# ZwwWayne/mmMOT

Hardware: NVIDIA H100
Metric: frame-pairs/sec at N=128 dets (higher is better)
Workload: dtype f32 (tensor-core engine: FP16 hi/lo split operands, fp32 accumulate)

## Files before the change

### mmmot_b200/csrc/gemm_tma.cuh

```cuda
#pragma once
#include <cuda.h>
#include <cuda_fp16.h>

#include "tc_common.cuh"

namespace tma {

using namespace tc;

constexpr int T_THREADS = 384;
constexpr int T_EPI_WARPS = 8, T_LOAD_WARP = 8;
constexpr int T_CONS_REGS = 232, T_LOAD_REGS = 40;
static_assert(256 * T_CONS_REGS + 128 * T_LOAD_REGS <= launch_regs(T_THREADS) * T_THREADS, "register split exceeds the CTA's pool");
constexpr int T_EPI_SCRATCH = 32 * 80;
constexpr int T_STAGES = 4;
constexpr int T_STAGE_BYTES = A_SUB + 2 * B_HALF;
constexpr size_t T_SMEM_BYTES = (size_t)T_STAGES * T_STAGE_BYTES + 1024 + 256 + T_EPI_WARPS * T_EPI_SCRATCH;
static_assert(T_SMEM_BYTES <= 227 * 1024, "gemm_tma_kernel exceeds the 227 KB of shared memory per block");
static_assert(T_STAGES * T_STAGE_BYTES >= 128 * BN * 4, "the accumulator image must fit in the ring it overlays");

enum { OUT_PLANAR = 3 };

struct TmaP {
  TcP t;
  int conv;
  int bx, by, bi;
  int tiles_x, tiles_y;
  int n_img, H, W, C;
  long plane_elems;
  int ksegs, kc_per_seg;
  float* acc_scratch;
  int halo, pool;
  unsigned long long* pool_sum;
  unsigned long long* segsum;
  int* status;
  int wcompact;
  const float* gen_src;
  const int4* chunk_tab;
};

static __global__ void seg_chunk_tab_kernel(const int4* __restrict__ tiles, int num_tiles, const int* __restrict__ seg,
                                            int4* __restrict__ tab) {
  const int idx = blockIdx.x * blockDim.x + threadIdx.x;
  if (idx >= num_tiles * 2) return;
  const int4 tt = tiles[idx >> 1];
  const int half = idx & 1, c0 = tt.y, len = tt.z;
  int v[4];
#pragma unroll
  for (int c = 0; c < 4; c++) {
    const int col0 = half * 128 + c * 32;
    v[c] = 0;
    if (col0 < len) {
      const int first = seg[c0 + col0], last = seg[c0 + min(col0 + 31, len - 1)];
      v[c] = (first << 1) | ((col0 + 32 <= len && first == last) ? 1 : 0);
    }
  }
  tab[idx] = make_int4(v[0], v[1], v[2], v[3]);
}

__device__ __forceinline__ void tma_load_2d(uint32_t dst, const CUtensorMap* map, int c0, int c1, uint32_t mbar) {
  asm volatile(
      "cp.async.bulk.tensor.2d.shared::cluster.global.tile.mbarrier::complete_tx::bytes [%0], [%1, {%2, %3}], [%4];"
      ::"r"(dst), "l"(reinterpret_cast<uint64_t>(map)), "r"(c0), "r"(c1), "r"(mbar)
      : "memory");
}
__device__ __forceinline__ void tma_load_4d(uint32_t dst, const CUtensorMap* map, int c0, int c1, int c2, int c3,
                                            uint32_t mbar) {
  asm volatile(
      "cp.async.bulk.tensor.4d.shared::cluster.global.tile.mbarrier::complete_tx::bytes [%0], [%1, {%2, %3, %4, %5}], "
      "[%6];"
      ::"r"(dst), "l"(reinterpret_cast<uint64_t>(map)), "r"(c0), "r"(c1), "r"(c2), "r"(c3), "r"(mbar)
      : "memory");
}
__device__ __forceinline__ uint64_t smem_desc_sw64(uint32_t saddr) {
  return (uint64_t)((saddr & 0x3FFFFu) >> 4) | ((uint64_t)1 << 16) | ((uint64_t)(512 >> 4) << 32) | (2ull << 62);
}
__device__ __forceinline__ void st_global_256(void* dst, const uint4& a, const uint4& b) {
  asm volatile("st.global.v4.b32 [%0], {%1, %2, %3, %4};\n\tst.global.v4.b32 [%0+16], {%5, %6, %7, %8};" ::"l"(dst),
               "r"(a.x), "r"(a.y), "r"(a.z), "r"(a.w), "r"(b.x), "r"(b.y), "r"(b.z), "r"(b.w)
               : "memory");
}
__device__ __forceinline__ void st_global_256(void* dst, const uint32_t* r) {
  st_global_256(dst, make_uint4(r[0], r[1], r[2], r[3]), make_uint4(r[4], r[5], r[6], r[7]));
}
__device__ __forceinline__ void split_f16(float x, __half& hi, __half& lo) {
  unsigned short a, b;
  asm("{\n\t.reg .f32 f;\n\t"
      "cvt.rn.satfinite.f16.f32 %0, %2;\n\t"
      "cvt.f32.f16 f, %0;\n\t"
      "sub.f32 f, %2, f;\n\t"
      "cvt.rn.satfinite.f16.f32 %1, f;\n\t}"
      : "=h"(a), "=h"(b)
      : "f"(x));
  hi = __ushort_as_half(a);
  lo = __ushort_as_half(b);
}

template <int BX>
__device__ __forceinline__ void pool_chunk(const float (&x)[32], float (&o)[8]) {
#pragma unroll
  for (int a = 0; a < 16 / BX; a++)
#pragma unroll
    for (int b = 0; b < BX / 2; b++) {
      const int i = 2 * a * BX + 2 * b;
      o[a * (BX / 2) + b] = fmaxf(fmaxf(x[i], x[i + 1]), fmaxf(x[i + BX], x[i + BX + 1]));
    }
}

static __global__ void __launch_bounds__(T_THREADS, 1)
gemm_tma_kernel(const TmaP P, const __grid_constant__ CUtensorMap map_hi, const __grid_constant__ CUtensorMap map_lo) {
  const GemmP& p = P.t.g;
  extern __shared__ uint8_t smem_raw[];
  const uint32_t raw = smem_u32(smem_raw);
  const uint32_t base = (raw + 1023u) & ~1023u;
  uint8_t* sm = smem_raw + (base - raw);
  const uint32_t bar0 = base + T_STAGES * T_STAGE_BYTES;
  auto full_bar = [&](int s) { return bar0 + 8u * s; };
  auto empty_bar = [&](int s) { return bar0 + 8u * (T_STAGES + s); };
  const uint32_t free_bar = bar0 + 8u * (2 * T_STAGES);
  float* img = reinterpret_cast<float*>(sm);
  uint8_t* epi_scratch = sm + T_STAGES * T_STAGE_BYTES + 256;

  const int tid = threadIdx.x, warp = tid >> 5, lane = tid & 31;
  const int mgroups = P.t.m_tiles;
  const long total_tiles = (long)p.num_tiles * mgroups;
  const int KC = P.t.k_chunks;
  const int cchunks = P.conv ? P.C / BK : KC;

  if (tid == 0) {
    for (int s = 0; s < T_STAGES; s++) {
      mbar_init(full_bar(s), 1);
      mbar_init(empty_bar(s), T_EPI_WARPS);
    }
    mbar_init(free_bar, T_EPI_WARPS);
    asm volatile("fence.mbarrier_init.release.cluster;" ::: "memory");
  }
  __syncthreads();

  auto tile_cols = [&](int nt, int& g, int& c0, int& len) {
    if (p.tile_tab) { int4 tt = p.tile_tab[nt]; g = tt.x; c0 = tt.y; len = tt.z; }
    else { g = nt / p.tiles_per_group; c0 = (nt - g * p.tiles_per_group) * BN; len = min(BN, p.S - c0); }
  };
  auto conv_origin = [&](int nt, int& i0, int& y0, int& x0) {
    const int tx = nt % P.tiles_x;
    const int r = nt / P.tiles_x;
    const int ty = r % P.tiles_y;
    i0 = (r / P.tiles_y) * P.bi; y0 = ty * P.by; x0 = tx * P.bx;
  };

  if (warp < T_EPI_WARPS) {
    asm volatile("setmaxnreg.inc.sync.aligned.u32 %0;" ::"n"(T_CONS_REGS));
    const int q = warp & 3, half = warp >> 2;
    const int lbx = 31 - __clz(max(P.bx, 1)), lby = 31 - __clz(max(P.by, 1));
    uint32_t wcount = 0;
    uint32_t it = 0;
    float acc[2][64];
    float amax = 0.f;
    __half* yh = reinterpret_cast<__half*>(p.Y);
    __half* scr = reinterpret_cast<__half*>(epi_scratch + warp * T_EPI_SCRATCH);
    auto store_rows = [&](const float (&x)[32], bool ok, long o) {
      __half h[32], l[32];
#pragma unroll
      for (int j = 0; j < 32; j++) { split_f16(x[j], h[j], l[j]); amax = fmaxf(amax, fabsf(x[j])); }
#pragma unroll
      for (int pl = 0; pl < 2; pl++) {
#pragma unroll
        for (int j = 0; j < 32; j++) scr[j * 40 + lane] = pl ? l[j] : h[j];
        __syncwarp();
        if (ok) {
          const uint4* src = reinterpret_cast<const uint4*>(scr + lane * 40);
          __half* dst = yh + o + (pl ? P.plane_elems : 0);
          const uint4 a = src[0], b = src[1], c = src[2], d = src[3];
          st_global_256(dst, a, b);
          st_global_256(dst + 16, c, d);
        }
        __syncwarp();
      }
    };
    auto store_planar_block = [&](const float (&x)[32], int col0, int cb, int i0, int y0, int x0) {
      const int col = col0 + lane;
      const int xx = col & (P.bx - 1), r = col >> lbx;
      const int yy = r & (P.by - 1), ii = r >> lby;
      const int img = i0 + ii, y = y0 + yy, xg = x0 + xx;
      store_rows(x, img < P.n_img && y < P.H && xg < P.W, (((long)img * P.H + y) * P.W + xg) * p.y_ms + cb);
    };
    const int Hp = P.H >> 1, Wp = P.W >> 1;
    float hprev[16];
    float psum = 0.f;
    int psum_img = -1;
    auto pool_flush = [&](int co_) {
      if (P.pool_sum && psum_img >= 0 && psum_img < P.n_img)
        atomicAdd(P.pool_sum + (long)psum_img * p.M + co_, __float2ull_rn(psum * 4294967296.f));
      psum = 0.f; psum_img = -1;
    };
    auto pool_emit = [&](const float (&o)[16], int np, int r0, int rstep_q, int wq, int cb, int co_, int i0, int y0, int x0) {
      float xs[32];
#pragma unroll
      for (int j = 0; j < 32; j++) xs[j] = j < 16 ? o[j] : 0.f;
      const int q = lane < np ? lane : 0;
      const int r = r0 + 2 * (q / wq), xx = 2 * (q - (q / wq) * wq);
      const int yy = r & (P.by - 1), ii = r >> lby;
      const int img = i0 + ii, y = y0 + yy, xg = x0 + xx;
      const bool ok = lane < np && img < P.n_img && y < P.H && xg < P.W;
      store_rows(xs, ok, (((long)img * Hp + (y >> 1)) * Wp + (xg >> 1)) * p.y_ms + cb);
      if (P.pool_sum) {
        (void)rstep_q;
#pragma unroll
        for (int j = 0; j < 16; j++) {
          if (j < np) {
            const int rj = r0 + 2 * (j / wq), xj = 2 * (j - (j / wq) * wq);
            const int imj = i0 + (rj >> lby);
            const bool okj = imj < P.n_img && y0 + (rj & (P.by - 1)) < P.H && x0 + xj < P.W;
            if (imj != psum_img) { pool_flush(co_); psum_img = imj; }
            if (okj) psum += o[j];
          }
        }
      }
    };
    auto emit_conv = [&](const float (&x)[32], int cc, int col0, int co_, int i0, int y0, int x0) {
      if (!P.pool) { store_planar_block(x, col0, co_ - lane, i0, y0, x0); return; }
      float o[16];
      const int r0 = col0 >> lbx;
      if (P.bx == 32) {
        if (!(cc & 1)) {
#pragma unroll
          for (int b = 0; b < 16; b++) hprev[b] = fmaxf(x[2 * b], x[2 * b + 1]);
          return;
        }
#pragma unroll
        for (int b = 0; b < 16; b++) o[b] = fmaxf(hprev[b], fmaxf(x[2 * b], x[2 * b + 1]));
        pool_emit(o, 16, r0 - 1, 0, 16, co_ - lane, co_, i0, y0, x0);
        return;
      }
      float o8[8];
      if (P.bx == 16) pool_chunk<16>(x, o8);
      else if (P.bx == 8) pool_chunk<8>(x, o8);
      else if (P.bx == 4) pool_chunk<4>(x, o8);
      else pool_chunk<2>(x, o8);
#pragma unroll
      for (int j = 0; j < 16; j++) o[j] = j < 8 ? o8[j] : 0.f;
      pool_emit(o, 8, r0, 0, P.bx >> 1, co_ - lane, co_, i0, y0, x0);
    };

    for (long t = blockIdx.x; t < total_tiles; t += gridDim.x) {
      const int mg = (int)(t % mgroups);
      const int nt = (int)(t / mgroups);
      int g = 0, c0 = 0, len = BN, i0 = 0, y0 = 0, x0 = 0;
      if (P.conv) conv_origin(nt, i0, y0, x0); else tile_cols(nt, g, c0, len);
      for (int seg = 0; seg < P.ksegs; seg++, wcount++) {
#pragma unroll
      for (int mb = 0; mb < 2; mb++)
#pragma unroll
        for (int i = 0; i < 64; i++) acc[mb][i] = 0.f;
      const int kc_lo = seg * P.kc_per_seg, kc_hi = min(KC, kc_lo + P.kc_per_seg);
      for (int kc = kc_lo; kc < kc_hi; kc++, it++) {
        const int s = it % T_STAGES;
        mbar_wait(full_bar(s), (it / T_STAGES) & 1);
        const uint32_t sa = base + s * T_STAGE_BYTES, sb = sa + A_SUB + half * (128 / 8) * 512;
        if (!(P.t.dbg & 8)) {
          wgmma_fence();
#pragma unroll
          for (int ks = 0; ks < 2; ks++) {
            const uint64_t b_hi = smem_desc_sw64(sb + ks * 32), b_lo = smem_desc_sw64(sb + B_HALF + ks * 32);
#pragma unroll
            for (int mb = 0; mb < 2; mb++) {
              const uint32_t a = sa + mb * 8 * SBO + ks * 2 * A_LBO;
              const uint64_t a_hi = smem_desc(a, A_LBO, SBO), a_lo = smem_desc(a + A_HALF, A_LBO, SBO);
              wgmma_n128(acc[mb], a_hi, b_hi, ((kc - kc_lo) | ks) ? 1u : 0u);
              wgmma_n128(acc[mb], a_hi, b_lo, 1u);
              wgmma_n128(acc[mb], a_lo, b_hi, 1u);
            }
          }
          wgmma_commit();
        }
        wgmma_wait<1>();
        if (kc > kc_lo) { __syncwarp(); if (lane == 0) mbar_arrive(empty_bar((it - 1) % T_STAGES)); }
      }
      wgmma_wait<0>();
      fence_acc(acc[0]);
      fence_acc(acc[1]);
      __syncwarp();
      if (lane == 0) mbar_arrive(empty_bar((it - 1) % T_STAGES));
      bar_sync(7, T_EPI_WARPS * 32);
      acc_dump(acc[0], img, BN, 0, half * 128);
      acc_dump(acc[1], img, BN, 64, half * 128);
      bar_sync(7, T_EPI_WARPS * 32);
      if (P.ksegs > 1) {
        {
          const int co = mg * 128 + q * 32 + lane;
          const bool rowok = co < p.M;
          const float bv = (rowok && p.bias) ? __ldg(p.bias + co) : 0.f;
#pragma unroll 1
          for (int cc = 0; cc < 4; cc++) {
            const int col0 = half * 128 + cc * 32;
            uint32_t v[32];
            acc_ld32(img, BN, q * 32 + lane, col0, v);
            if (!rowok) continue;
            float* sp = P.acc_scratch + ((long)nt * BN + col0) * p.M + co;
            if (seg < P.ksegs - 1) {
              if (seg == 0) {
#pragma unroll
                for (int j = 0; j < 32; j++) __stcg(sp + (long)j * p.M, __uint_as_float(v[j]) * P.t.out_scale);
              } else {
                float sv[32];
#pragma unroll
                for (int j = 0; j < 32; j++) sv[j] = __ldcg(sp + (long)j * p.M);
#pragma unroll
                for (int j = 0; j < 32; j++) __stcg(sp + (long)j * p.M, fmaf(__uint_as_float(v[j]), P.t.out_scale, sv[j]));
              }
            } else {
              float sv[32];
#pragma unroll
              for (int j = 0; j < 32; j++) sv[j] = __ldcg(sp + (long)j * p.M);
#pragma unroll
              for (int j = 0; j < 32; j++) {
                float a = fmaf(__uint_as_float(v[j]), P.t.out_scale, sv[j]) + bv;
                sv[j] = p.relu ? fmaxf(a, 0.f) : a;
              }
              emit_conv(sv, cc, col0, co, i0, y0, x0);
            }
          }
          if (P.pool && seg == P.ksegs - 1 && rowok) pool_flush(co);
        }
      } else
      {
        const int co = mg * 128 + q * 32 + lane;
        const bool rowok = co < p.M;
        const float bv = (rowok && p.bias) ? __ldg(p.bias + co) : 0.f;
        double f1 = 0.0, f2 = 0.0;
        const bool pass2 = P.segsum && !p.part && !p.Y && !p.relu;
        const bool use_seg = p.seg && (p.addend || P.segsum);
        int4 ct = make_int4(0, 0, 0, 0);
        if (use_seg) ct = __ldg(P.chunk_tab + (long)nt * 2 + half);
        const int cdesc[4] = {ct.x, ct.y, ct.z, ct.w};
        float adv[4] = {0.f, 0.f, 0.f, 0.f};
        unsigned one_det = 0;
#pragma unroll
        for (int c = 0; c < 4; c++) {
          if (cdesc[c] & 1) {
            one_det |= 1u << c;
            if (p.addend && rowok) adv[c] = __ldg(p.addend + (long)(cdesc[c] >> 1) * p.ld_add + co);
          }
        }
        float na = 0.f, nb = 0.f;
        if (P.segsum && rowok) { na = __ldg(p.sc + (long)g * p.M + co); nb = __ldg(p.sh + (long)g * p.M + co); }
#pragma unroll 1
        for (int cc = 0; cc < 4; cc++) {
          const int col0 = half * 128 + cc * 32;
          if (col0 >= len) break;
          const int da = (cc == 0 ? ct.x : cc == 1 ? ct.y : cc == 2 ? ct.z : ct.w) >> 1;
          const float adc = cc == 0 ? adv[0] : cc == 1 ? adv[1] : cc == 2 ? adv[2] : adv[3];
          const bool single = (one_det >> cc) & 1u;
          uint32_t v[32];
          acc_ld32(img, BN, q * 32 + lane, col0, v);
          if (P.t.dbg & 1) continue;
          float s1 = 0.f, s2 = 0.f, pv = 0.f;
          bool fast = col0 + 32 <= len;
          if (pass2 && fast) {
            if (single) {
              if (rowok) {
                const float bva = bv + adc;
                const float a2 = P.t.out_scale * na, b2 = fmaf(bva, na, nb);
                float r0 = 0.f, r1 = 0.f;
#pragma unroll
                for (int j = 0; j < 32; j += 2) {
                  r0 += fmaxf(fmaf(__uint_as_float(v[j]), a2, b2), 0.f);
                  r1 += fmaxf(fmaf(__uint_as_float(v[j + 1]), a2, b2), 0.f);
                }
                atomicAdd(P.segsum + (long)da * p.M + co, __float2ull_rn((r0 + r1) * 4294967296.f));
              }
              continue;
            }
          }
          float bva = bv;
          if (fast && p.addend) {
            if (single) bva += adc;
            else fast = false;
          }
          if (fast) {
            if (p.relu) epi_fast<true>(v, P.t.out_scale, bva, pv, s1, s2);
            else epi_fast<false>(v, P.t.out_scale, bva, pv, s1, s2);
          } else {
            float t = 0.f;
#pragma unroll
            for (int j = 0; j < 32; j++) {
              float x = fmaf(__uint_as_float(v[j]), P.t.out_scale, bv);
              const int col = col0 + j;
              if (p.addend && rowok && col < len)
                x += __ldg(p.addend + (long)__ldg(p.seg + c0 + col) * p.ld_add + co);
              if (p.relu) x = fmaxf(x, 0.f);
              v[j] = __float_as_uint(x);
              if (col < len) t += x;
            }
            pv = t / (float)min(32, len - col0);
#pragma unroll
            for (int j = 0; j < 32; j++)
              if (col0 + j < len) { const float d = __uint_as_float(v[j]) - pv; s1 += d; s2 = fmaf(d, d, s2); }
          }
          stat_fold(f1, f2, min(32, len - col0), pv, s1, s2);
          if (P.segsum && rowok) {
            const int nvalid = min(32, len - col0);
            int dcur = da;
            float run = 0.f;
            if (single) {
#pragma unroll
              for (int j = 0; j < 32; j++) run += fmaxf(fmaf(__uint_as_float(v[j]), na, nb), 0.f);
            } else {
#pragma unroll
              for (int j = 0; j < 32; j++) {
                if (j < nvalid) {
                  const int d = __ldg(p.seg + c0 + col0 + j);
                  if (d != dcur) {
                    atomicAdd(P.segsum + (long)dcur * p.M + co, __float2ull_rn(run * 4294967296.f));
                    run = 0.f; dcur = d;
                  }
                  run += fmaxf(fmaf(__uint_as_float(v[j]), na, nb), 0.f);
                }
              }
            }
            atomicAdd(P.segsum + (long)dcur * p.M + co, __float2ull_rn(run * 4294967296.f));
          }
          if (!p.Y || !rowok) continue;
          if (P.conv) {
            float xv[32];
#pragma unroll
            for (int j = 0; j < 32; j++) xv[j] = __uint_as_float(v[j]);
            emit_conv(xv, cc, col0, co, i0, y0, x0);
          } else {
            const int nvalid = min(32, len - col0);
            const long row0 = (long)g * p.y_gs + c0 + col0;
            if (P.t.out_mode == OUT_PLANAR && !(p.y_ms & 31)) {
              float xv[32];
#pragma unroll
              for (int j = 0; j < 32; j++) xv[j] = __uint_as_float(v[j]);
              store_rows(xv, lane < nvalid, (row0 + lane) * p.y_ms + (co - lane));
            } else if (P.t.out_mode == OUT_PLANAR) {
              __half* dst = yh + row0 * p.y_ms + co;
#pragma unroll
              for (int j = 0; j < 32; j++)
                if (j < nvalid) {
                  __half h, l;
                  split_f16(__uint_as_float(v[j]), h, l);
                  amax = fmaxf(amax, fabsf(__uint_as_float(v[j])));
                  dst[(long)j * p.y_ms] = h;
                  dst[(long)j * p.y_ms + P.plane_elems] = l;
                }
            } else {
              float* dst = p.Y + row0 * p.y_ms + co;
              if (nvalid == 32) {
#pragma unroll
                for (int j = 0; j < 32; j++) { *dst = __uint_as_float(v[j]); dst += p.y_ms; }
              } else {
#pragma unroll
                for (int j = 0; j < 32; j++)
                  if (j < nvalid) dst[(long)j * p.y_ms] = __uint_as_float(v[j]);
              }
            }
          }
        }
        if (p.part && rowok) p.part[((long)nt * 2 + half) * p.M + co] = make_double2(f1, f2);
        if (P.conv && P.pool && rowok) pool_flush(co);
      }
      fence_async_smem();
      __syncwarp();
      if (lane == 0) mbar_arrive(free_bar);
      }
    }
    mm_range_flag(P.status, amax);
  } else {
    asm volatile("setmaxnreg.dec.sync.aligned.u32 %0;" ::"n"(T_LOAD_REGS));
    if (warp == T_LOAD_WARP && lane == 0) {
      uint32_t it = 0, wcount = 0;
      for (long t = blockIdx.x; t < total_tiles; t += gridDim.x) {
        const int mg = (int)(t % mgroups);
        const int nt = (int)(t / mgroups);
        const int mt0 = mg;
        int g = 0, c0 = 0, len = BN, i0 = 0, y0 = 0, x0 = 0;
        if (P.conv) conv_origin(nt, i0, y0, x0); else tile_cols(nt, g, c0, len);
        const int row0 = (int)((long)g * p.x_gs + c0);
        for (int kc = 0; kc < KC; kc++, it++) {
          if (kc % P.kc_per_seg == 0) {
            if (wcount > 0) mbar_wait(free_bar, (wcount - 1) & 1);
            wcount++;
          }
          const int s = it % T_STAGES;
          mbar_wait(empty_bar(s), ((it / T_STAGES) & 1) ^ 1);
          const uint32_t abytes = (uint32_t)A_SUB;
          const bool skipA = P.t.dbg & 2, skipB = P.t.dbg & 4;
          mbar_expect_tx(full_bar(s), (skipA ? 0u : abytes) + (skipB ? 0u : 2u * B_HALF));
          const uint32_t sa = base + s * T_STAGE_BYTES, sb = sa + A_SUB;
          const uint8_t* src = reinterpret_cast<const uint8_t*>(P.t.Wp) + ((size_t)kc * P.t.m_tiles + mt0) * A_SUB;
          if (!skipA) bulk_g2s(sa, src, abytes, full_bar(s));
          if (skipB) continue;
          if (P.conv) {
            const int tap = kc / cchunks, cc = kc - tap * cchunks;
            const int dx = tap % 3 - 1, dy = tap / 3 - 1;
            tma_load_4d(sb, &map_hi, cc * BK, x0 + dx, y0 + dy, i0, full_bar(s));
            tma_load_4d(sb + B_HALF, &map_lo, cc * BK, x0 + dx, y0 + dy, i0, full_bar(s));
          } else {
            tma_load_2d(sb, &map_hi, kc * BK, row0, full_bar(s));
            tma_load_2d(sb + B_HALF, &map_lo, kc * BK, row0, full_bar(s));
          }
        }
      }
    }
    __syncwarp();
  }

}

typedef CUresult (*EncodeTiledFn)(CUtensorMap*, CUtensorMapDataType, cuuint32_t, void*, const cuuint64_t*,
                                  const cuuint64_t*, const cuuint32_t*, const cuuint32_t*, CUtensorMapInterleave,
                                  CUtensorMapSwizzle, CUtensorMapL2promotion, CUtensorMapFloatOOBfill);
static inline EncodeTiledFn encode_fn() {
  static EncodeTiledFn fn = nullptr;
  if (!fn) {
    void* p = nullptr;
    cudaDriverEntryPointQueryResult qr;
    if (cudaGetDriverEntryPoint("cuTensorMapEncodeTiled", &p, cudaEnableDefault, &qr) == cudaSuccess &&
        qr == cudaDriverEntryPointSuccess)
      fn = (EncodeTiledFn)p;
  }
  return fn;
}
static inline int make_map_2d(CUtensorMap* m, const void* basep, long rows, int C, long ld) {
  EncodeTiledFn fn = encode_fn();
  if (!fn) return MMMOT_E_ARG;
  cuuint64_t dims[2] = {(cuuint64_t)C, (cuuint64_t)rows};
  cuuint64_t strides[1] = {(cuuint64_t)ld * 2};
  cuuint32_t box[2] = {32, 256}, es[2] = {1, 1};
  CUresult r = fn(m, CU_TENSOR_MAP_DATA_TYPE_FLOAT16, 2, const_cast<void*>(basep), dims, strides, box, es,
                  CU_TENSOR_MAP_INTERLEAVE_NONE, CU_TENSOR_MAP_SWIZZLE_64B, CU_TENSOR_MAP_L2_PROMOTION_L2_128B,
                  CU_TENSOR_MAP_FLOAT_OOB_FILL_NONE);
  return r == CUDA_SUCCESS ? 0 : 900 + (int)r;
}
static inline int make_map_2d_f32(CUtensorMap* m, const void* basep, long rows, int C, int box_rows,
                                  CUtensorMapSwizzle swizzle) {
  EncodeTiledFn fn = encode_fn();
  if (!fn) return MMMOT_E_ARG;
  cuuint64_t dims[2] = {(cuuint64_t)C, (cuuint64_t)rows};
  cuuint64_t strides[1] = {(cuuint64_t)C * 4};
  cuuint32_t box[2] = {32, (cuuint32_t)box_rows}, es[2] = {1, 1};
  CUresult r = fn(m, CU_TENSOR_MAP_DATA_TYPE_FLOAT32, 2, const_cast<void*>(basep), dims, strides, box, es,
                  CU_TENSOR_MAP_INTERLEAVE_NONE, swizzle, CU_TENSOR_MAP_L2_PROMOTION_L2_128B,
                  CU_TENSOR_MAP_FLOAT_OOB_FILL_NONE);
  return r == CUDA_SUCCESS ? 0 : 900 + (int)r;
}
static inline int make_map_4d(CUtensorMap* m, const void* basep, int n_img, int H, int W, int C, int bx, int by,
                              int bi) {
  EncodeTiledFn fn = encode_fn();
  if (!fn) return MMMOT_E_ARG;
  cuuint64_t dims[4] = {(cuuint64_t)C, (cuuint64_t)W, (cuuint64_t)H, (cuuint64_t)n_img};
  cuuint64_t strides[3] = {(cuuint64_t)C * 2, (cuuint64_t)W * C * 2, (cuuint64_t)H * W * C * 2};
  cuuint32_t box[4] = {32, (cuuint32_t)bx, (cuuint32_t)by, (cuuint32_t)bi}, es[4] = {1, 1, 1, 1};
  CUresult r = fn(m, CU_TENSOR_MAP_DATA_TYPE_FLOAT16, 4, const_cast<void*>(basep), dims, strides, box, es,
                  CU_TENSOR_MAP_INTERLEAVE_NONE, CU_TENSOR_MAP_SWIZZLE_64B, CU_TENSOR_MAP_L2_PROMOTION_L2_128B,
                  CU_TENSOR_MAP_FLOAT_OOB_FILL_NONE);
  return r == CUDA_SUCCESS ? 0 : 900 + (int)r;
}

}

#include "gemm_tma_px.cuh"

static int gemm_tma_px_launch(tma::TmaP& P, const CUtensorMap& mh, const CUtensorMap& ml, int sms, cudaStream_t st) {
  static std::atomic<unsigned long long> attr{0};
  MM_TRY(mm_ensure_smem(tma::gemm_tma_px_kernel<false>, tma::PX_SMEM_BYTES, attr));
  const long total = P.t.g.num_tiles;
  const int grid = (int)(total < sms ? total : sms);
  tma::gemm_tma_px_kernel<false><<<grid, tma::PX_THREADS, tma::PX_SMEM_BYTES, st>>>(P, mh, ml);
  MM_LAUNCH_CHECK();
  return 0;
}

static int gemm_tma_px_launch_gen27(const float* crops, int n_img, int H, int W, const uint4* Wpx, float out_scale,
                                    const float* bias, __half* Yhi, long y_plane, int* status, cudaStream_t st) {
  if (!crops || !Wpx || !Yhi) return MMMOT_E_ARG;
  const long n_pix = (long)n_img * H * W;
  if (n_pix >= (1L << 31) || ((long)H * W) % tc::BN || (tc::BN + 2 * W + 2) * 12 > 2 * tma::PX_W_SLOT) return MMMOT_E_SHAPE;
  int sms = 0;
  MM_TRY(mm_sm_count(&sms));
  static std::atomic<unsigned long long> attr{0};
  MM_TRY(mm_ensure_smem(tma::gemm_tma_px_kernel<true>, tma::PX_SMEM_BYTES, attr));
  tma::TmaP P;
  memset(&P, 0, sizeof(P));
  GemmP g = gemm_defaults();
  g.bias = bias; g.M = 64; g.K = 32; g.relu = 1;
  g.S = (int)n_pix; g.tiles_per_group = mm_cdiv(n_pix, tc::BN); g.num_tiles = g.tiles_per_group;
  g.Y = reinterpret_cast<float*>(Yhi); g.y_ms = 64;
  P.t.g = g;
  P.t.Wp = Wpx; P.wcompact = 1;
  P.t.m_tiles = 1; P.t.k_chunks = 1;
  P.t.out_scale = out_scale;
  P.t.out_mode = tma::OUT_PLANAR;
  P.t.dbg = mm_debug_flags();
  P.plane_elems = y_plane;
  P.ksegs = 1; P.kc_per_seg = 1;
  P.status = status;
  P.gen_src = crops; P.n_img = n_img; P.H = H; P.W = W;
  alignas(64) CUtensorMap dummy;
  memset(&dummy, 0, sizeof(dummy));
  const long total = g.num_tiles;
  const int grid = (int)(total < sms ? total : sms);
  tma::gemm_tma_px_kernel<true><<<grid, tma::PX_GEN_THREADS, tma::PX_SMEM_BYTES, st>>>(P, dummy, dummy);
  MM_LAUNCH_CHECK();
  return 0;
}

static int gemm_tma_launch_mat(const GemmP& g, const uint4* Wp, float out_scale, const __half* Xhi, long x_plane,
                               long rows, int ldx, int out_mode, long y_plane, cudaStream_t st,
                               unsigned long long* segsum = nullptr, int* status = nullptr, const int4* chunk_tab = nullptr,
                               const uint4* Wpx = nullptr) {
  if (!Wp || g.num_tiles <= 0 || g.K % tc::BK) return MMMOT_E_ARG;
  int sms = 0;
  MM_TRY(mm_sm_count(&sms));
  static std::atomic<unsigned long long> attr{0};
  MM_TRY(mm_ensure_smem(tma::gemm_tma_kernel, tma::T_SMEM_BYTES, attr));
  tma::TmaP P;
  memset(&P, 0, sizeof(P));
  P.t.g = g;
  P.t.Wp = Wp;
  P.t.m_tiles = (g.M + 127) / 128;
  P.t.k_chunks = g.K / tc::BK;
  P.t.out_scale = out_scale;
  P.t.out_mode = out_mode;
  P.t.dbg = mm_debug_flags();
  P.plane_elems = y_plane;
  P.ksegs = 1; P.kc_per_seg = P.t.k_chunks;
  P.segsum = segsum;
  P.status = status;
  P.chunk_tab = chunk_tab;
  if (g.seg && (g.addend || segsum) && !chunk_tab) return MMMOT_E_ARG;
  alignas(64) CUtensorMap mh, ml;
  MM_TRY(tma::make_map_2d(&mh, Xhi, rows, g.K, ldx));
  MM_TRY(tma::make_map_2d(&ml, Xhi + x_plane, rows, g.K, ldx));
  if (out_mode == tma::OUT_PLANAR && g.M == 64 && g.y_ms == 64 && !g.part && !segsum && !g.addend && !g.tile_tab &&
      !(P.t.dbg & 64)) {
    if (Wpx) { P.t.Wp = Wpx; P.wcompact = 1; }
    return gemm_tma_px_launch(P, mh, ml, sms, st);
  }
  const long total = (long)g.num_tiles * P.t.m_tiles;
  const int grid = (int)(total < sms ? total : sms);
  tma::gemm_tma_kernel<<<grid, tma::T_THREADS, tma::T_SMEM_BYTES, st>>>(P, mh, ml);
  MM_LAUNCH_CHECK();
  return 0;
}

static inline double conv_box_waste(int n_img, int H, int W, int bx, int by, int bi) {
  return (double)mm_cdiv(W, bx) * bx / W * mm_cdiv(H, by) * by / H * mm_cdiv(n_img, bi) * bi / n_img;
}

struct ConvPlan {
  int px;
  int halo;
  int pool;
  int bx, by, bi;
  int ksegs, kc_per_seg;
  int tiles_x, tiles_y, num_tiles;
};
static inline ConvPlan conv_plan(int M, bool part, int n_img, int H, int W, int C, bool want_pool, bool use_kseg, int dbg,
                                 int seg_chunks) {
  ConvPlan c;
  memset(&c, 0, sizeof(c));
  c.bx = 1; c.by = 1; c.bi = 256;
  double best = 1e30;
  for (int cx = 256; cx >= 1; cx >>= 1)
    for (int cy = 256 / cx; cy >= 1; cy >>= 1) {
      const int ci = 256 / (cx * cy);
      const double waste = conv_box_waste(n_img, H, W, cx, cy, ci);
      if (waste < best - 1e-9) { best = waste; c.bx = cx; c.by = cy; c.bi = ci; }
    }
  const int kchunks = 9 * C / tc::BK;
  c.px = M == 64 && !part && !(dbg & 64) && !(use_kseg && seg_chunks > 0 && kchunks > seg_chunks);
  if (c.px && conv_box_waste(1, H, W, 16, 16, 1) <= best + 1e-9) { c.bx = 16; c.by = 16; c.bi = 1; }
  if (c.px) {
    c.halo = (c.bi == 1 && c.bx >= 8 && c.bx * (c.by + 2) * 64 <= tma::PX_X_PLANE && !(dbg & 256)) ? 1 : 0;
    c.pool = want_pool && c.bx >= 2 && c.bx <= 16 && c.by >= 2 && !(H & 1) && !(W & 1) && !(dbg & 512);
  } else {
    c.pool = want_pool && c.bx >= 2 && c.bx <= 32 && c.by >= 2 && !(H & 1) && !(W & 1) && !(dbg & 512);
  }
  c.ksegs = 1; c.kc_per_seg = kchunks;
  if (use_kseg && seg_chunks > 0 && kchunks > seg_chunks) {
    c.ksegs = (kchunks + seg_chunks - 1) / seg_chunks;
    c.kc_per_seg = (kchunks + c.ksegs - 1) / c.ksegs;
  }
  c.tiles_x = mm_cdiv(W, c.bx); c.tiles_y = mm_cdiv(H, c.by);
  c.num_tiles = c.tiles_x * c.tiles_y * mm_cdiv(n_img, c.bi);
  return c;
}

static int gemm_tma_launch_conv(const GemmP& g0, const uint4* Wp, float out_scale, const __half* Xhi, long x_plane,
                                int n_img, int H, int W, int C, __half* Yhi, long y_plane, cudaStream_t st,
                                float* acc_scratch = nullptr, long y_plane_pooled = 0, int* did_pool = nullptr,
                                int* status = nullptr, unsigned long long* pool_sum = nullptr, const uint4* Wpx = nullptr,
                                ConvPlan* plan = nullptr) {
  if (did_pool) *did_pool = 0;
  if (!Wp || C % tc::BK) return MMMOT_E_ARG;
  const ConvPlan c = conv_plan(g0.M, g0.part != nullptr, n_img, H, W, C, y_plane_pooled > 0 && did_pool,
                               acc_scratch != nullptr, mm_debug_flags(), mm_kseg_chunks());
  if (plan) *plan = c;
  int sms = 0;
  MM_TRY(mm_sm_count(&sms));
  static std::atomic<unsigned long long> attr{0};
  MM_TRY(mm_ensure_smem(tma::gemm_tma_kernel, tma::T_SMEM_BYTES, attr));
  tma::TmaP P;
  memset(&P, 0, sizeof(P));
  GemmP g = g0;
  g.K = 9 * C;
  P.conv = 1; P.bx = c.bx; P.by = c.by; P.bi = c.bi;
  P.halo = c.halo;
  P.pool = c.pool;
  if (c.pool) *did_pool = 1;
  if (c.pool && !c.px) P.pool_sum = pool_sum;
  P.tiles_x = c.tiles_x; P.tiles_y = c.tiles_y;
  P.n_img = n_img; P.H = H; P.W = W; P.C = C;
  g.num_tiles = c.num_tiles;
  g.tile_tab = nullptr;
  g.Y = reinterpret_cast<float*>(Yhi);
  g.y_ms = g.M;
  P.t.g = g;
  P.t.Wp = Wp;
  P.t.m_tiles = (g.M + 127) / 128;
  P.t.k_chunks = g.K / tc::BK;
  P.t.out_scale = out_scale;
  P.t.out_mode = tma::OUT_PLANAR;
  P.t.dbg = mm_debug_flags();
  P.plane_elems = P.pool ? y_plane_pooled : y_plane;
  P.status = status;
  P.ksegs = c.ksegs; P.kc_per_seg = c.kc_per_seg;
  if (c.ksegs > 1) P.acc_scratch = acc_scratch;
  alignas(64) CUtensorMap mh, ml;
  const int box_y = P.halo ? c.by + 2 : c.by;
  MM_TRY(tma::make_map_4d(&mh, Xhi, n_img, H, W, C, c.bx, box_y, c.bi));
  MM_TRY(tma::make_map_4d(&ml, Xhi + x_plane, n_img, H, W, C, c.bx, box_y, c.bi));
  if (c.px) {
    if (Wpx) { P.t.Wp = Wpx; P.wcompact = 1; }
    return gemm_tma_px_launch(P, mh, ml, sms, st);
  }
  const long total = (long)g.num_tiles * P.t.m_tiles;
  const int grid = (int)(total < sms ? total : sms);
  tma::gemm_tma_kernel<<<grid, tma::T_THREADS, tma::T_SMEM_BYTES, st>>>(P, mh, ml);
  MM_LAUNCH_CHECK();
  return 0;
}
```

### mmmot_b200/csrc/gemm_tma_px.cuh

```cuda
#pragma once

namespace tma {

constexpr int PX_W_SLOT = 8192;
constexpr int PX_W_LBO = 1024;
constexpr int PX_X_OFF = 3 * PX_W_SLOT;
constexpr int PX_X_PLANE = 24576;
constexpr int PX_STAGE = PX_X_OFF + 2 * PX_X_PLANE;
constexpr int PX_STAGES = 2;
constexpr int PX_IMG = 256 * 64 * 4;
constexpr size_t PX_SMEM_BYTES = (size_t)PX_STAGES * PX_STAGE + PX_IMG + 1024 + 256;

constexpr int PX_WC_LBO = 2048;

constexpr int PX_THREADS = 288, PX_GEN_THREADS = 640, PX_GEN_WARP0 = 12;
constexpr int PX_CONS_REGS = 144, PX_LOAD_REGS = 24, PX_PROD_REGS = 80;
static_assert(256 * PX_CONS_REGS + 128 * PX_LOAD_REGS + 256 * PX_PROD_REGS <= launch_regs(PX_GEN_THREADS) * PX_GEN_THREADS,
              "GEN27 register split exceeds the CTA's pool");

constexpr int PX_GEN_WARPS = 4;

template <bool GEN27>
static __global__ void __launch_bounds__(GEN27 ? PX_GEN_THREADS : PX_THREADS, 1)
gemm_tma_px_kernel(const TmaP P, const __grid_constant__ CUtensorMap map_hi, const __grid_constant__ CUtensorMap map_lo) {
  const GemmP& p = P.t.g;
  extern __shared__ uint8_t smem_raw[];
  __shared__ float s_bias[64];
  const uint32_t raw = smem_u32(smem_raw);
  const uint32_t base = (raw + 1023u) & ~1023u;
  uint8_t* sm = smem_raw + (base - raw);
  float* img = reinterpret_cast<float*>(sm + PX_STAGES * PX_STAGE);
  const uint32_t bar0 = base + PX_STAGES * PX_STAGE + PX_IMG;
  auto full_bar = [&](int s) { return bar0 + 8u * s; };
  auto empty_bar = [&](int s) { return bar0 + 8u * (PX_STAGES + s); };

  const int tid = threadIdx.x, warp = tid >> 5, lane = tid & 31;
  const long total_tiles = p.num_tiles;
  const int KC = P.t.k_chunks;
  const int cchunks = P.conv ? P.C / BK : KC;
  const int ntap = P.halo ? 3 : 1;
  const int nstage = P.halo ? 3 * cchunks : KC;
  const uint32_t xbytes = P.halo ? (uint32_t)(P.bx * (P.by + 2) * 64) : (uint32_t)B_HALF;

  if (tid < 64) s_bias[tid] = p.bias ? p.bias[tid] : 0.f;
  if (tid == 0) {
    for (int s = 0; s < PX_STAGES; s++) {
      mbar_init(full_bar(s), GEN27 ? 1 + PX_GEN_WARPS : 1);
      mbar_init(empty_bar(s), T_EPI_WARPS);
    }
    asm volatile("fence.mbarrier_init.release.cluster;" ::: "memory");
  }
  __syncthreads();

  auto conv_origin = [&](int nt, int& i0, int& y0, int& x0) {
    const int tx = nt % P.tiles_x;
    const int r = nt / P.tiles_x;
    const int ty = r % P.tiles_y;
    i0 = (r / P.tiles_y) * P.bi; y0 = ty * P.by; x0 = tx * P.bx;
  };

  if (warp < T_EPI_WARPS) {
    if (GEN27) asm volatile("setmaxnreg.inc.sync.aligned.u32 %0;" ::"n"(PX_CONS_REGS));
    const int q = warp & 3, cb = (warp >> 2) * 32;
    const int lbx = 31 - __clz(max(P.bx, 1)), lby = 31 - __clz(max(P.by, 1));
    __half* yh = reinterpret_cast<__half*>(p.Y);
    uint32_t racc = 0;
    uint32_t it = 0;
    const int wg = warp >> 2;
    float acc[2][32];
#pragma unroll
    for (int mb = 0; mb < 2; mb++)
#pragma unroll
      for (int i = 0; i < 32; i++) acc[mb][i] = 0.f;
    for (long t = blockIdx.x; t < total_tiles; t += gridDim.x) {
      const int nt = (int)t;
      int i0 = 0, y0 = 0, x0 = 0;
      if (P.conv) conv_origin(nt, i0, y0, x0);
      for (int si = 0; si < nstage; si++, it++) {
        const int s = it % PX_STAGES;
        mbar_wait(full_bar(s), (it / PX_STAGES) & 1);
        const uint32_t sw = base + s * PX_STAGE, sx = sw + PX_X_OFF;
        if (!(P.t.dbg & 8)) {
          wgmma_fence();
          for (int ky = 0; ky < ntap; ky++) {
            const uint32_t xo = sx + (uint32_t)(ky * P.bx * 64 + wg * (128 * 64)), wo = sw + (uint32_t)(ky * PX_W_SLOT);
#pragma unroll
            for (int ks = 0; ks < 2; ks++) {
              uint64_t w_hi, w_lo;
              if (P.wcompact) {
                w_hi = smem_desc(wo + ks * 2 * PX_WC_LBO, PX_WC_LBO, SBO);
                w_lo = smem_desc(wo + 8 * SBO + ks * 2 * PX_WC_LBO, PX_WC_LBO, SBO);
              } else {
                w_hi = smem_desc(wo + ks * 2 * PX_W_LBO, PX_W_LBO, SBO);
                w_lo = smem_desc(wo + PX_W_SLOT / 2 + ks * 2 * PX_W_LBO, PX_W_LBO, SBO);
              }
#pragma unroll
              for (int mb = 0; mb < 2; mb++) {
                const uint64_t x_hi = smem_desc_sw64(xo + mb * (64 * 64) + ks * 32);
                const uint64_t x_lo = smem_desc_sw64(xo + PX_X_PLANE + mb * (64 * 64) + ks * 32);
                wgmma_n64(acc[mb], x_hi, w_hi, (si | ky | ks) ? 1u : 0u);
                wgmma_n64(acc[mb], x_hi, w_lo, 1u);
                wgmma_n64(acc[mb], x_lo, w_hi, 1u);
              }
            }
          }
          wgmma_commit();
        }
        wgmma_wait<1>();
        if (si > 0) { __syncwarp(); if (lane == 0) mbar_arrive(empty_bar((it - 1) % PX_STAGES)); }
      }
      wgmma_wait<0>();
      fence_acc(acc[0]);
      fence_acc(acc[1]);
      __syncwarp();
      if (lane == 0) mbar_arrive(empty_bar((it - 1) % PX_STAGES));
      bar_sync(7, T_EPI_WARPS * 32);
      acc_dump(acc[0], img, 64, wg * 128, 0);
      acc_dump(acc[1], img, 64, wg * 128 + 64, 0);
      bar_sync(7, T_EPI_WARPS * 32);
#pragma unroll 1
      for (int sub = 0; sub < 2; sub++) {
        const int col = sub * 128 + q * 32 + lane;
        bool ok;
        long o;
        if (P.conv) {
          const int xx = col & (P.bx - 1), r = col >> lbx;
          const int yy = r & (P.by - 1), ii = r >> lby;
          const int img = i0 + ii, y = y0 + yy, xg = x0 + xx;
          ok = img < P.n_img && y < P.H && xg < P.W;
          o = (((long)img * P.H + y) * P.W + xg) * 64 + cb;
        } else {
          const long row = (long)nt * BN + col;
          ok = row < p.S;
          o = row * 64 + cb;
        }
        uint32_t v[32];
        acc_ld32(img, 64, sub * 128 + q * 32 + lane, cb, v);
        if (P.t.dbg & 1) continue;
        if (P.pool) {
#pragma unroll
          for (int j = 0; j < 32; j++) {
            float a = __uint_as_float(v[j]);
            a = fmaxf(a, __shfl_xor_sync(0xffffffffu, a, 1));
            a = fmaxf(a, __shfl_xor_sync(0xffffffffu, a, P.bx));
            v[j] = __float_as_uint(a);
          }
          const int xx = col & (P.bx - 1), r = col >> lbx;
          const int yy = r & (P.by - 1);
          const int y = y0 + yy, xg = x0 + xx;
          ok = ok && !(xx & 1) && !(yy & 1);
          o = (((long)(i0 + (r >> lby)) * (P.H >> 1) + (y >> 1)) * (P.W >> 1) + (xg >> 1)) * 64 + cb;
          if (!ok) continue;
        }
        uint32_t hi[16], lo[16];
#pragma unroll
        for (int j = 0; j < 32; j += 2) {
          float x0v = fmaf(__uint_as_float(v[j]), P.t.out_scale, s_bias[cb + j]);
          float x1v = fmaf(__uint_as_float(v[j + 1]), P.t.out_scale, s_bias[cb + j + 1]);
          if (p.relu) { x0v = fmaxf(x0v, 0.f); x1v = fmaxf(x1v, 0.f); }
          split_f16x2(x0v, x1v, hi[j >> 1], lo[j >> 1]);
          mm_range_track2(racc, hi[j >> 1]);
        }
        if (GEN27) {
          const uint32_t scr = base + (uint32_t)((q >> 1) * PX_STAGE + PX_X_OFF + (q & 1) * PX_X_PLANE + 16384);
          const uint32_t rowa = scr + (uint32_t)lane * 128u;
#pragma unroll
          for (int k = 0; k < 4; k++) {
            const uint32_t slot = (uint32_t)((((cb >> 3) + k) ^ (lane & 7)) << 4);
            asm volatile("st.shared.v4.b32 [%0], {%1, %2, %3, %4};" ::"r"(rowa + slot), "r"(hi[4 * k]), "r"(hi[4 * k + 1]),
                         "r"(hi[4 * k + 2]), "r"(hi[4 * k + 3]) : "memory");
            asm volatile("st.shared.v4.b32 [%0], {%1, %2, %3, %4};" ::"r"(rowa + 4096u + slot), "r"(lo[4 * k]),
                         "r"(lo[4 * k + 1]), "r"(lo[4 * k + 2]), "r"(lo[4 * k + 3]) : "memory");
          }
          asm volatile("bar.sync %0, 64;" ::"r"(3 + q) : "memory");
          const int h = warp >> 2;
          const long row0 = (long)nt * BN + sub * 128 + q * 32;
          __half* dstp = yh + (long)h * P.plane_elems + row0 * 64;
#pragma unroll
          for (int r = 0; r < 4; r++) {
            const int idx = r * 32 + lane, px = idx >> 2, c = (idx & 3) * 2;
            const uint32_t ra = scr + (uint32_t)h * 4096u + (uint32_t)px * 128u;
            uint32_t w[8];
            asm volatile("ld.shared.v4.b32 {%0, %1, %2, %3}, [%4];" : "=r"(w[0]), "=r"(w[1]), "=r"(w[2]), "=r"(w[3])
                         : "r"(ra + (uint32_t)((c ^ (px & 7)) << 4)));
            asm volatile("ld.shared.v4.b32 {%0, %1, %2, %3}, [%4];" : "=r"(w[4]), "=r"(w[5]), "=r"(w[6]), "=r"(w[7])
                         : "r"(ra + (uint32_t)(((c + 1) ^ (px & 7)) << 4)));
            if (row0 + px < p.S) st_global_256(dstp + (long)px * 64 + c * 8, w);
          }
          asm volatile("bar.sync %0, 64;" ::"r"(3 + q) : "memory");
        } else if (ok && !(P.t.dbg & 128)) {
          st_global_256(yh + o, hi);
          st_global_256(yh + o + 16, hi + 8);
          st_global_256(yh + o + P.plane_elems, lo);
          st_global_256(yh + o + P.plane_elems + 16, lo + 8);
        } else if (ok) {
          uint4* dh = reinterpret_cast<uint4*>(yh + o);
          uint4* dl = reinterpret_cast<uint4*>(yh + o + P.plane_elems);
#pragma unroll
          for (int k = 0; k < 4; k++) {
            dh[k] = make_uint4(hi[4 * k], hi[4 * k + 1], hi[4 * k + 2], hi[4 * k + 3]);
            dl[k] = make_uint4(lo[4 * k], lo[4 * k + 1], lo[4 * k + 2], lo[4 * k + 3]);
          }
        }
      }
    }
    mm_range_flag2(P.status, racc);
  } else if (GEN27 && warp >= PX_GEN_WARP0) {
    asm volatile("setmaxnreg.dec.sync.aligned.u32 %0;" ::"n"(PX_PROD_REGS));
    const int pw = warp - PX_GEN_WARP0;
    const int grp = pw >> 2;
    const int pt = (pw & 3) * 32 + lane;
    const int W = P.W, hw = P.H * P.W;
    const int span = BN + 2 * W + 2;
    float amax = 0.f;
    uint32_t it = (uint32_t)grp;
    for (long t = blockIdx.x + (long)grp * gridDim.x; t < total_tiles; t += 2L * gridDim.x, it += 2) {
      const int s = it % PX_STAGES;
      const long row0 = t * BN;
      const long img = row0 / hw;
      const int r0 = (int)(row0 - img * hw);
      const float* src = P.gen_src + img * 3 * hw;
      mbar_wait(empty_bar(s), ((it / PX_STAGES) & 1) ^ 1);
      float* stg = reinterpret_cast<float*>(sm + s * PX_STAGE + PX_W_SLOT);
      const int lin0 = r0 - W - 1;
      if (P.t.dbg & 4) {
        __syncwarp();
        if (lane == 0) mbar_arrive(full_bar(s));
        continue;
      }
#pragma unroll 1
      for (int i0 = pt; i0 < 3 * span; i0 += 8 * 128) {
        float q[8];
#pragma unroll
        for (int u = 0; u < 8; u++) {
          const int i = i0 + u * 128;
          const int ci = i / span, lin = lin0 + (i - ci * span);
          q[u] = (i < 3 * span && lin >= 0 && lin < hw) ? __ldg(src + (long)ci * hw + lin) : 0.f;
        }
#pragma unroll
        for (int u = 0; u < 8; u++)
          if (i0 + u * 128 < 3 * span) stg[i0 + u * 128] = q[u];
      }
      asm volatile("bar.sync %0, 128;" ::"r"(1 + grp) : "memory");
      const uint32_t sx = base + s * PX_STAGE + PX_X_OFF;
#pragma unroll
      for (int j = 0; j < 2; j++) {
        const int rr = j * 128 + pt;
        const int x = (r0 + rr) % W;
        const bool xl = x > 0, xr = x < W - 1;
        const float* c = stg + rr + W + 1;
        float v[28];
#pragma unroll
        for (int ci = 0; ci < 3; ci++)
#pragma unroll
          for (int ky = 0; ky < 3; ky++)
#pragma unroll
            for (int kx = 0; kx < 3; kx++) {
              float q = c[ci * span + (ky - 1) * W + (kx - 1)];
              if (kx == 0 && !xl) q = 0.f;
              if (kx == 2 && !xr) q = 0.f;
              v[ci * 9 + ky * 3 + kx] = q;
              amax = fmaxf(amax, fabsf(q));
            }
        v[27] = 0.f;
        uint32_t hi[16], lo[16];
#pragma unroll
        for (int k = 0; k < 28; k += 2) split_f16x2(v[k], v[k + 1], hi[k >> 1], lo[k >> 1]);
        hi[14] = hi[15] = lo[14] = lo[15] = 0u;
        const uint32_t rowaddr = sx + (uint32_t)rr * 64u, sw = (uint32_t)((rr >> 1) & 3);
#pragma unroll
        for (int cch = 0; cch < 4; cch++) {
          const uint32_t a = rowaddr + ((cch ^ sw) << 4);
          asm volatile("st.shared.v4.b32 [%0], {%1, %2, %3, %4};" ::"r"(a), "r"(hi[4 * cch]), "r"(hi[4 * cch + 1]),
                       "r"(hi[4 * cch + 2]), "r"(hi[4 * cch + 3]) : "memory");
          asm volatile("st.shared.v4.b32 [%0], {%1, %2, %3, %4};" ::"r"(a + PX_X_PLANE), "r"(lo[4 * cch]),
                       "r"(lo[4 * cch + 1]), "r"(lo[4 * cch + 2]), "r"(lo[4 * cch + 3]) : "memory");
        }
      }
      asm volatile("fence.proxy.async.shared::cta;" ::: "memory");
      __syncwarp();
      if (lane == 0) mbar_arrive(full_bar(s));
    }
    mm_range_flag(P.status, amax);
  } else {
    if (GEN27) asm volatile("setmaxnreg.dec.sync.aligned.u32 %0;" ::"n"(PX_LOAD_REGS));
    if (warp == T_LOAD_WARP && lane == 0) {
      uint32_t it = 0;
      for (long t = blockIdx.x; t < total_tiles; t += gridDim.x) {
        const int nt = (int)t;
        int i0 = 0, y0 = 0, x0 = 0;
        if (P.conv) conv_origin(nt, i0, y0, x0);
        for (int si = 0; si < nstage; si++, it++) {
          const int s = it % PX_STAGES;
          mbar_wait(empty_bar(s), ((it / PX_STAGES) & 1) ^ 1);
          mbar_expect_tx(full_bar(s), (uint32_t)ntap * PX_W_SLOT + (GEN27 ? 0u : 2u * xbytes));
          const uint32_t sw = base + s * PX_STAGE, sx = sw + PX_X_OFF;
          const int kx = P.halo ? si / cchunks : 0, cc = P.halo ? si - kx * cchunks : 0;
          for (int ky = 0; ky < ntap; ky++) {
            const int kc = P.halo ? (ky * 3 + kx) * cchunks + cc : si;
            if (P.wcompact) {
              bulk_g2s(sw + ky * PX_W_SLOT, reinterpret_cast<const uint8_t*>(P.t.Wp) + (size_t)kc * PX_W_SLOT, PX_W_SLOT, full_bar(s));
            } else {
              const uint8_t* src = reinterpret_cast<const uint8_t*>(P.t.Wp) + (size_t)kc * P.t.m_tiles * A_SUB;
#pragma unroll
              for (int r = 0; r < 8; r++)
                bulk_g2s(sw + ky * PX_W_SLOT + r * PX_W_LBO, src + r * A_LBO, 1024, full_bar(s));
            }
          }
          if (P.halo) {
            tma_load_4d(sx, &map_hi, cc * BK, x0 + kx - 1, y0 - 1, i0, full_bar(s));
            tma_load_4d(sx + PX_X_PLANE, &map_lo, cc * BK, x0 + kx - 1, y0 - 1, i0, full_bar(s));
          } else if (P.conv) {
            const int tap = si / cchunks, c2 = si - tap * cchunks;
            const int dx = tap % 3 - 1, dy = tap / 3 - 1;
            tma_load_4d(sx, &map_hi, c2 * BK, x0 + dx, y0 + dy, i0, full_bar(s));
            tma_load_4d(sx + PX_X_PLANE, &map_lo, c2 * BK, x0 + dx, y0 + dy, i0, full_bar(s));
          } else if (!GEN27) {
            tma_load_2d(sx, &map_hi, si * BK, nt * BN, full_bar(s));
            tma_load_2d(sx + PX_X_PLANE, &map_lo, si * BK, nt * BN, full_bar(s));
          }
        }
      }
    }
    __syncwarp();
  }
}

}
```

Before: 195.4.

## Deepen px kernel pipeline to three stages with halved epilogue staging image

Shrinks the X plane and the accumulator staging image so a third TMA pipeline stage fits in shared memory for the non-GEN27 path. The epilogue now dumps one warpgroup's accumulators at a time into a half-size image, with extra barriers per sub-tile. HALO becomes a template parameter so the tap loop is unrolled at compile time, and debug skip flags are added to the loader. The GEN27 path stays at two stages and its scratch region is relocated into the third stage area. The risks are the added epilogue serialization and the reduced X plane size constraining halo box sizes.

```diff
diff --git a/mmmot_b200/csrc/gemm_tma.cuh b/mmmot_b200/csrc/gemm_tma.cuh
--- a/mmmot_b200/csrc/gemm_tma.cuh
+++ b/mmmot_b200/csrc/gemm_tma.cuh
@@ -564,11 +564,12 @@
 #include "gemm_tma_px.cuh"
 
 static int gemm_tma_px_launch(tma::TmaP& P, const CUtensorMap& mh, const CUtensorMap& ml, int sms, cudaStream_t st) {
-  static std::atomic<unsigned long long> attr{0};
-  MM_TRY(mm_ensure_smem(tma::gemm_tma_px_kernel<false>, tma::PX_SMEM_BYTES, attr));
+  static std::atomic<unsigned long long> attr[2];
+  const auto kernel = P.halo ? tma::gemm_tma_px_kernel<false, true> : tma::gemm_tma_px_kernel<false, false>;
+  MM_TRY(mm_ensure_smem(kernel, tma::PX_SMEM_BYTES, attr[P.halo ? 1 : 0]));
   const long total = P.t.g.num_tiles;
   const int grid = (int)(total < sms ? total : sms);
-  tma::gemm_tma_px_kernel<false><<<grid, tma::PX_THREADS, tma::PX_SMEM_BYTES, st>>>(P, mh, ml);
+  kernel<<<grid, tma::PX_THREADS, tma::PX_SMEM_BYTES, st>>>(P, mh, ml);
   MM_LAUNCH_CHECK();
   return 0;
 }
@@ -581,7 +582,7 @@
   int sms = 0;
   MM_TRY(mm_sm_count(&sms));
   static std::atomic<unsigned long long> attr{0};
-  MM_TRY(mm_ensure_smem(tma::gemm_tma_px_kernel<true>, tma::PX_SMEM_BYTES, attr));
+  MM_TRY(mm_ensure_smem(tma::gemm_tma_px_kernel<true, false>, tma::PX_SMEM_BYTES, attr));
   tma::TmaP P;
   memset(&P, 0, sizeof(P));
   GemmP g = gemm_defaults();
@@ -602,7 +603,7 @@
   memset(&dummy, 0, sizeof(dummy));
   const long total = g.num_tiles;
   const int grid = (int)(total < sms ? total : sms);
-  tma::gemm_tma_px_kernel<true><<<grid, tma::PX_GEN_THREADS, tma::PX_SMEM_BYTES, st>>>(P, dummy, dummy);
+  tma::gemm_tma_px_kernel<true, false><<<grid, tma::PX_GEN_THREADS, tma::PX_SMEM_BYTES, st>>>(P, dummy, dummy);
   MM_LAUNCH_CHECK();
   return 0;
 }
diff --git a/mmmot_b200/csrc/gemm_tma_px.cuh b/mmmot_b200/csrc/gemm_tma_px.cuh
--- a/mmmot_b200/csrc/gemm_tma_px.cuh
+++ b/mmmot_b200/csrc/gemm_tma_px.cuh
@@ -5,11 +5,12 @@
 constexpr int PX_W_SLOT = 8192;
 constexpr int PX_W_LBO = 1024;
 constexpr int PX_X_OFF = 3 * PX_W_SLOT;
-constexpr int PX_X_PLANE = 24576;
+constexpr int PX_X_PLANE = 20480;
 constexpr int PX_STAGE = PX_X_OFF + 2 * PX_X_PLANE;
-constexpr int PX_STAGES = 2;
-constexpr int PX_IMG = 256 * 64 * 4;
+constexpr int PX_STAGES = 3;
+constexpr int PX_IMG = 128 * 64 * 4;
 constexpr size_t PX_SMEM_BYTES = (size_t)PX_STAGES * PX_STAGE + PX_IMG + 1024 + 256;
+static_assert(PX_SMEM_BYTES <= 227 * 1024, "px kernel exceeds the shared memory of an SM");
 
 constexpr int PX_WC_LBO = 2048;
 
@@ -20,9 +21,10 @@
 
 constexpr int PX_GEN_WARPS = 4;
 
-template <bool GEN27>
+template <bool GEN27, bool HALO>
 static __global__ void __launch_bounds__(GEN27 ? PX_GEN_THREADS : PX_THREADS, 1)
 gemm_tma_px_kernel(const TmaP P, const __grid_constant__ CUtensorMap map_hi, const __grid_constant__ CUtensorMap map_lo) {
+  static_assert(!(GEN27 && HALO), "GEN27 tiles are not halo boxes");
   const GemmP& p = P.t.g;
   extern __shared__ uint8_t smem_raw[];
   __shared__ float s_bias[64];
@@ -31,6 +33,7 @@
   uint8_t* sm = smem_raw + (base - raw);
   float* img = reinterpret_cast<float*>(sm + PX_STAGES * PX_STAGE);
   const uint32_t bar0 = base + PX_STAGES * PX_STAGE + PX_IMG;
+  constexpr int NST = GEN27 ? 2 : PX_STAGES;
   auto full_bar = [&](int s) { return bar0 + 8u * s; };
   auto empty_bar = [&](int s) { return bar0 + 8u * (PX_STAGES + s); };
 
@@ -38,13 +41,13 @@
   const long total_tiles = p.num_tiles;
   const int KC = P.t.k_chunks;
   const int cchunks = P.conv ? P.C / BK : KC;
-  const int ntap = P.halo ? 3 : 1;
-  const int nstage = P.halo ? 3 * cchunks : KC;
-  const uint32_t xbytes = P.halo ? (uint32_t)(P.bx * (P.by + 2) * 64) : (uint32_t)B_HALF;
+  constexpr int ntap = HALO ? 3 : 1;
+  const int nstage = HALO ? 3 * cchunks : KC;
+  const uint32_t xbytes = HALO ? (uint32_t)(P.bx * (P.by + 2) * 64) : (uint32_t)B_HALF;
 
   if (tid < 64) s_bias[tid] = p.bias ? p.bias[tid] : 0.f;
   if (tid == 0) {
-    for (int s = 0; s < PX_STAGES; s++) {
+    for (int s = 0; s < NST; s++) {
       mbar_init(full_bar(s), GEN27 ? 1 + PX_GEN_WARPS : 1);
       mbar_init(empty_bar(s), T_EPI_WARPS);
     }
@@ -77,11 +80,12 @@
       int i0 = 0, y0 = 0, x0 = 0;
       if (P.conv) conv_origin(nt, i0, y0, x0);
       for (int si = 0; si < nstage; si++, it++) {
-        const int s = it % PX_STAGES;
-        mbar_wait(full_bar(s), (it / PX_STAGES) & 1);
+        const int s = it % NST;
+        mbar_wait(full_bar(s), (it / NST) & 1);
         const uint32_t sw = base + s * PX_STAGE, sx = sw + PX_X_OFF;
         if (!(P.t.dbg & 8)) {
           wgmma_fence();
+#pragma unroll
           for (int ky = 0; ky < ntap; ky++) {
             const uint32_t xo = sx + (uint32_t)(ky * P.bx * 64 + wg * (128 * 64)), wo = sw + (uint32_t)(ky * PX_W_SLOT);
 #pragma unroll
@@ -107,19 +111,21 @@
           wgmma_commit();
         }
         wgmma_wait<1>();
-        if (si > 0) { __syncwarp(); if (lane == 0) mbar_arrive(empty_bar((it - 1) % PX_STAGES)); }
+        if (si > 0) { __syncwarp(); if (lane == 0) mbar_arrive(empty_bar((it - 1) % NST)); }
       }
       wgmma_wait<0>();
       fence_acc(acc[0]);
       fence_acc(acc[1]);
       __syncwarp();
-      if (lane == 0) mbar_arrive(empty_bar((it - 1) % PX_STAGES));
-      bar_sync(7, T_EPI_WARPS * 32);
-      acc_dump(acc[0], img, 64, wg * 128, 0);
-      acc_dump(acc[1], img, 64, wg * 128 + 64, 0);
-      bar_sync(7, T_EPI_WARPS * 32);
+      if (lane == 0) mbar_arrive(empty_bar((it - 1) % NST));
 #pragma unroll 1
       for (int sub = 0; sub < 2; sub++) {
+        bar_sync(7, T_EPI_WARPS * 32);
+        if (wg == sub) {
+          acc_dump(acc[0], img, 64, 0, 0);
+          acc_dump(acc[1], img, 64, 64, 0);
+        }
+        bar_sync(7, T_EPI_WARPS * 32);
         const int col = sub * 128 + q * 32 + lane;
         bool ok;
         long o;
@@ -135,7 +141,7 @@
           o = row * 64 + cb;
         }
         uint32_t v[32];
-        acc_ld32(img, 64, sub * 128 + q * 32 + lane, cb, v);
+        acc_ld32(img, 64, q * 32 + lane, cb, v);
         if (P.t.dbg & 1) continue;
         if (P.pool) {
 #pragma unroll
@@ -162,7 +168,7 @@
           mm_range_track2(racc, hi[j >> 1]);
         }
         if (GEN27) {
-          const uint32_t scr = base + (uint32_t)((q >> 1) * PX_STAGE + PX_X_OFF + (q & 1) * PX_X_PLANE + 16384);
+          const uint32_t scr = base + (uint32_t)(2 * PX_STAGE + q * 8192);
           const uint32_t rowa = scr + (uint32_t)lane * 128u;
 #pragma unroll
           for (int k = 0; k < 4; k++) {
@@ -215,12 +221,12 @@
     float amax = 0.f;
     uint32_t it = (uint32_t)grp;
     for (long t = blockIdx.x + (long)grp * gridDim.x; t < total_tiles; t += 2L * gridDim.x, it += 2) {
-      const int s = it % PX_STAGES;
+      const int s = it % NST;
       const long row0 = t * BN;
       const long img = row0 / hw;
       const int r0 = (int)(row0 - img * hw);
       const float* src = P.gen_src + img * 3 * hw;
-      mbar_wait(empty_bar(s), ((it / PX_STAGES) & 1) ^ 1);
+      mbar_wait(empty_bar(s), ((it / NST) & 1) ^ 1);
       float* stg = reinterpret_cast<float*>(sm + s * PX_STAGE + PX_W_SLOT);
       const int lin0 = r0 - W - 1;
       if (P.t.dbg & 4) {
@@ -291,13 +297,14 @@
         int i0 = 0, y0 = 0, x0 = 0;
         if (P.conv) conv_origin(nt, i0, y0, x0);
         for (int si = 0; si < nstage; si++, it++) {
-          const int s = it % PX_STAGES;
-          mbar_wait(empty_bar(s), ((it / PX_STAGES) & 1) ^ 1);
-          mbar_expect_tx(full_bar(s), (uint32_t)ntap * PX_W_SLOT + (GEN27 ? 0u : 2u * xbytes));
+          const int s = it % NST;
+          mbar_wait(empty_bar(s), ((it / NST) & 1) ^ 1);
+          const bool skipW = P.t.dbg & 2, skipX = GEN27 || (P.t.dbg & 4);
+          mbar_expect_tx(full_bar(s), (skipW ? 0u : (uint32_t)ntap * PX_W_SLOT) + (skipX ? 0u : 2u * xbytes));
           const uint32_t sw = base + s * PX_STAGE, sx = sw + PX_X_OFF;
-          const int kx = P.halo ? si / cchunks : 0, cc = P.halo ? si - kx * cchunks : 0;
-          for (int ky = 0; ky < ntap; ky++) {
-            const int kc = P.halo ? (ky * 3 + kx) * cchunks + cc : si;
+          const int kx = HALO ? si / cchunks : 0, cc = HALO ? si - kx * cchunks : 0;
+          for (int ky = 0; ky < ntap && !skipW; ky++) {
+            const int kc = HALO ? (ky * 3 + kx) * cchunks + cc : si;
             if (P.wcompact) {
               bulk_g2s(sw + ky * PX_W_SLOT, reinterpret_cast<const uint8_t*>(P.t.Wp) + (size_t)kc * PX_W_SLOT, PX_W_SLOT, full_bar(s));
             } else {
@@ -307,7 +314,8 @@
                 bulk_g2s(sw + ky * PX_W_SLOT + r * PX_W_LBO, src + r * A_LBO, 1024, full_bar(s));
             }
           }
-          if (P.halo) {
+          if (skipX) continue;
+          if (HALO) {
             tma_load_4d(sx, &map_hi, cc * BK, x0 + kx - 1, y0 - 1, i0, full_bar(s));
             tma_load_4d(sx + PX_X_PLANE, &map_lo, cc * BK, x0 + kx - 1, y0 - 1, i0, full_bar(s));
           } else if (P.conv) {
@@ -315,7 +323,7 @@
             const int dx = tap % 3 - 1, dy = tap / 3 - 1;
             tma_load_4d(sx, &map_hi, c2 * BK, x0 + dx, y0 + dy, i0, full_bar(s));
             tma_load_4d(sx + PX_X_PLANE, &map_lo, c2 * BK, x0 + dx, y0 + dy, i0, full_bar(s));
-          } else if (!GEN27) {
+          } else {
             tma_load_2d(sx, &map_hi, si * BK, nt * BN, full_bar(s));
             tma_load_2d(sx + PX_X_PLANE, &map_lo, si * BK, nt * BN, full_bar(s));
           }
```

Result: faster. 202.3 (median of 6 runs) (+3.5%).
